# NoelShin/PixelPick

Measured on AMD Instinct MI355X. Metric: train_step_throughput, higher is better.
Workload: dtype f32; 1 GPU; BASELINE configs[1]: Cityscapes 256x512, C=19, DeepLabv3+-MobileNetV2; train step per-GPU batch 4 with 20 labelled px/img + Adam; acquisition entropy top-k=20, B=256 images/launch/GPU, NCHW fp32 logits; global_batch=4

## Files before the change

include/pixelpick_hip_knobs.h:

```cpp
#ifndef PIXELPICK_HIP_KNOBS_H
#define PIXELPICK_HIP_KNOBS_H

void pp_debug_set_reduce_mode(int mode);
void pp_debug_set_exact_formula(int on);
void pp_debug_set_acq_tuning(int occ, int ppt);
void pp_debug_set_dw_variant(int v);
void pp_debug_set_splitk(int v);
void pp_debug_set_wgrad_target(int blocks);
void pp_debug_set_bn_target(int blocks);
void pp_debug_set_bn_bytes_per_block(int bytes);
void pp_debug_set_bn_probe(void* device_buffer);
void pp_debug_set_conv_thresholds(int v);
void pp_debug_conv_plan(int64_t M, int Cn, int Ck, int ntaps, int* out4);
void pp_debug_set_conv_rows(int bits);
void pp_debug_set_conv_bn_fuse(int bits);
void pp_debug_set_x3_variant(int v);
void pp_debug_set_gemm_pw(int v);
void pp_debug_set_x3f(int v);
void pp_debug_set_x3(int on);
void pp_debug_set_conv_variant(int v);
int pp_debug_launch_log(char* buf, int n);


int pp_debug_occupy_cus(int blocks, const int* stop, uint64_t max_ticks, uint64_t* started, pp_stream_t stream);


#endif
```

pixelpick_amd/_lib.py:

```python
import ctypes
import os
import struct

import torch

_HERE = os.path.dirname(os.path.abspath(__file__))
LIB_PATH = os.path.join(_HERE, "libpixelpick_hip.so")
KNOBS_LIB_PATH = os.path.join(_HERE, "libpixelpick_hip_knobs.so")
_use_knobs = [os.environ.get("PIXELPICK_KNOBS_BUILD", "0") not in ("", "0")]


def use_knobs_build(on: bool = True):
    if _lib is not None and _use_knobs[0] != bool(on):
        raise PixelPickHipError("use_knobs_build() after the library was loaded")
    _use_knobs[0] = bool(on)


def knobs_build() -> bool:
    return _use_knobs[0]

_i64, _p, _int, _sz, _f = ctypes.c_int64, ctypes.c_void_p, ctypes.c_int, ctypes.c_size_t, ctypes.c_float
_u64 = ctypes.c_uint64

SIGNATURES = {
# ... 83 lines not shown
    "pp_bilinear_bwd": (_int, [_p, _i64, _int, _int, _int, _int, _p, _i64, _int, _int, _int, _f, _f, _int, _p, _sz, _p]),
    "pp_image_colsum": (_int, [_p, _i64, _int, _i64, _int, _f, _p, _i64, _p]),
    "pp_image_broadcast": (_int, [_p, _i64, _int, _i64, _int, _f, _p, _i64, _p]),
    "pp_dropout": (_int, [_p, _i64, _p, _i64, _i64, _int, _f, ctypes.c_uint64, _p, _p]),
    "pp_dropout2d": (_int, [_p, _i64, _p, _i64, _int, _i64, _int, _f, ctypes.c_uint64, _p, _p]),
    "pp_aug_resample_h": (_int, [_p, _int, _int, _p, _p, _int, _int, _p, _p]),
    "pp_aug_vcrop": (_int, [_p, _p, _p] + [_int] * 11 + [_p, _p]),
    "pp_aug_labels": (_int, [_p, _p, _int, _p, _p, _p, _p] + [_int] * 8 + [_p, _p, _p]),
    "pp_aug_jitter": (_int, [_p, _i64, _int, _f, _p, _p]),
    "pp_aug_blur": (_int, [_p, _int, _int, _p, _int, _p, _p]),
    "pp_aug_blur_q8": (_int, [_p, _int, _int, _p, _int, _p, _p]),
    "pp_aug_to_tensor": (_int, [_p, _i64, ctypes.POINTER(_f), ctypes.POINTER(_f), _p, _p]),
    "pp_sparse_ce_workspace_bytes": (_sz, []),
    "pp_sparse_ce_fwd_bwd": (_int, [_p, _int, _int, _i64, _i64, _i64, _p, _int, _p, _p, _p, _p, _p, _sz, _p]),
    "pp_sparse_ce_lowres_workspace_bytes": (_sz, []),
    "pp_sparse_ce_lowres_fwd_bwd": (_int, [_p, _i64] + [_int] * 7 + [_p, _int, _p, _p, _p, _p, _i64, _p, _sz, _p]),
    "pp_confusion_matrix_update": (_int, [_p, _int, _int, _i64, _i64, _i64, _p, _p, _p]),
    "pp_adam_step_flat": (_int, [_p, _p, _p, _p, _i64, _i64, _f, _f, _f, _f, _f, _f, _i64, _f, _p, _p]),
    "pp_sgd_step_flat": (_int, [_p, _p, _p, _i64, _i64, _f, _f, _f, _f, _i64, _f, _p, _p]),
    "pp_add2d": (_int, [_p, _i64, _p, _i64, _p, _i64, _i64, _int, _p]),
    "pp_nhwc_to_nchw": (_int, [_p, _i64, _int, _int, _i64, _p, _p]),
    "pp_nchw_to_nhwc": (_int, [_p, _int, _int, _i64, _p, _i64, _p]),
    "pp_bn_fused_capacity": (_int, []),
    "pp_yardstick_stream_read": (_int, [_p, _sz, _int, _p, _p]),
    "pp_yardstick_mfma_stream": (_int, [_int, _int, _p, _p]),
    "pp_set_kernel_events": (None, [_p, _p, _int]),
    "pp_set_comm_cu_reserve": (None, [_int]),
    "pp_get_comm_cu_reserve": (_int, []),
    "pp_plan_create": (_p, []),
    "pp_plan_destroy": (None, [_p]),
    "pp_plan_size": (_i64, [_p]),
    "pp_plan_entry_args": (_int, [_p]),
    "pp_plan_add_call": (_int, [_p, _p, _p, _int]),
    "pp_plan_add_event_record": (_int, [_p, _p, _p]),
    "pp_plan_add_stream_wait": (_int, [_p, _p, _p]),
    "pp_plan_add_join": (_int, [_p, _p, _p]),
    "pp_plan_add_host_break": (_int, [_p]),
    "pp_plan_replay": (_int, [_p, _i64, ctypes.POINTER(_i64)]),
}

KNOB_SIGNATURES = {
    "pp_debug_set_reduce_mode": (None, [_int]),
    "pp_debug_set_exact_formula": (None, [_int]),
    "pp_debug_set_acq_tuning": (None, [_int, _int]),
    "pp_debug_set_dw_variant": (None, [_int]),
    "pp_debug_set_splitk": (None, [_int]),
    "pp_debug_set_wgrad_target": (None, [_int]),
    "pp_debug_set_bn_target": (None, [_int]),
    "pp_debug_set_bn_bytes_per_block": (None, [_int]),
    "pp_debug_set_bn_probe": (None, [_p]),
    "pp_debug_set_conv_thresholds": (None, [_int]),
    "pp_debug_conv_plan": (None, [_i64, _int, _int, _int, _p]),
    "pp_debug_set_conv_variant": (None, [_int]),
    "pp_debug_set_conv_rows": (None, [_int]),
    "pp_debug_set_conv_bn_fuse": (None, [_int]),
    "pp_debug_set_x3": (None, [_int]),
    "pp_debug_set_x3f": (None, [_int]),
    "pp_debug_set_gemm_pw": (None, [_int]),
    "pp_debug_set_x3_variant": (None, [_int]),
    "pp_debug_occupy_cus": (_int, [_int, _p, _u64, _p, _p]),
    "pp_debug_launch_log": (_int, [ctypes.c_char_p, _int]),
}

_lib = None
knob_epoch = [0]


def _knob_setter(fn):
    def setter(*args):
        knob_epoch[0] += 1
        return fn(*args)
    setter.__name__ = getattr(fn, "__name__", "pp_debug_set")
    setter.__wrapped__ = fn
    return setter


class PixelPickHipError(RuntimeError):
    pass


def _preload_torch_hip():
    tl = os.path.join(os.path.dirname(torch.__file__), "lib", "libamdhip64.so")
    if os.path.exists(tl):
        ctypes.CDLL(tl, mode=ctypes.RTLD_GLOBAL)


def lib():
    global _lib
    if _lib is None:
        path = KNOBS_LIB_PATH if _use_knobs[0] else LIB_PATH
        if not os.path.exists(path):
            raise PixelPickHipError(
                f"{path} not found: build the HIP extension first "
                f"(python -m pixelpick_amd.build, or __graft_entry__.build()). No fallback path exists.")
        _preload_torch_hip()
        L = ctypes.CDLL(path)
        sigs = dict(SIGNATURES)
        if _use_knobs[0]:
            sigs.update(KNOB_SIGNATURES)
        for name, (res, args) in sigs.items():
            fn = getattr(L, name)
            fn.restype = res
            fn.argtypes = args
            if name.startswith(("pp_debug_set_", "pp_set_comm")):
                setattr(L, name, _knob_setter(fn))
        _lib = L
# ... 256 lines not shown
```

pixelpick_amd/csrc/conv_igemm.hip:

```cpp
#include <atomic>
#include <type_traits>

#include "pp_common.h"
#include "bn_xchg.h"
#include "conv_types.h"

namespace pp {


static int g_conv_xcd_remap = 1;
static int g_conv_novec = 0;
static int g_conv_lds_pad = 0;
static int g_conv_variant = 0;

typedef float f32x16s __attribute__((ext_vector_type(16)));
constexpr int BK = 16;
struct __attribute__((packed, aligned(4))) StemF4 { float x, y, z, w; };
struct __attribute__((packed, aligned(4))) StemF3 { float x, y, z; };
struct __attribute__((packed, aligned(4))) StemF2 { float x, y; };


template <int TM, int TN, bool A_MK, bool B_NK, int PITCH_A, int PITCH_B, int BKT = BK>
__device__ __forceinline__ void mma_step(const float* As, const float* Bs, int a_row0, int b_col0, f32x16 (&acc)[TM][TN])
{
    const int lane = threadIdx.x & 63;
    const int l31 = lane & 31, h = lane >> 5;
    constexpr int NQ = BKT / 8;
    float a[NQ][TM][4], b[NQ][TN][4];
#pragma unroll
    for (int q = 0; q < NQ; ++q) {
        const int k0 = 8 * q + 4 * h;
#pragma unroll
        for (int tm = 0; tm < TM; ++tm) {
            const int r = a_row0 + tm * 32 + l31;
            if constexpr (A_MK) {
                const float4 v = *reinterpret_cast<const float4*>(As + r * PITCH_A + k0);
                a[q][tm][0] = v.x; a[q][tm][1] = v.y; a[q][tm][2] = v.z; a[q][tm][3] = v.w;
            } else {
#pragma unroll
                for (int j = 0; j < 4; ++j) a[q][tm][j] = As[(k0 + j) * PITCH_A + r];
            }
        }
#pragma unroll
        for (int tn = 0; tn < TN; ++tn) {
            const int c = b_col0 + tn * 32 + l31;
            if constexpr (B_NK) {
                const float4 v = *reinterpret_cast<const float4*>(Bs + c * PITCH_B + k0);
                b[q][tn][0] = v.x; b[q][tn][1] = v.y; b[q][tn][2] = v.z; b[q][tn][3] = v.w;
            } else {
#pragma unroll
                for (int j = 0; j < 4; ++j) b[q][tn][j] = Bs[(k0 + j) * PITCH_B + c];
            }
// ... 555 lines not shown
        }
    }
    const int64_t m0 = (int64_t)mt * BM;
    const int n0 = nt * BN;
    unsigned tag0 = 0;
    if constexpr (BNF) tag0 = tag_issue(p.bn.sync);
    const float* zero = g_zero16;
    asm volatile("" : "+v"(zero));
    const uint32_t lds0 = __builtin_amdgcn_readfirstlane((uint32_t)(uintptr_t)smem);

    int a_e0[PA], a_c[PA];
    unsigned a_vm[PA];
#pragma unroll
    for (int i = 0; i < PA; ++i) {
        const int row = (wave * PA + i) * 16 + (lane >> 2);
        a_c[i] = ((lane & 3) ^ ((row >> 2) & 3)) * 4;
        const int64_t m = m0 + row;
        a_e0[i] = 0;
        a_vm[i] = 0u;
        if (m < p.M) {
            const unsigned mu = (unsigned)m;
            const unsigned t = mu / (unsigned)p.Wo;
            const int ow = (int)(mu - t * (unsigned)p.Wo);
            const unsigned bb = t / (unsigned)p.Ho;
            const int oh = (int)(t - bb * (unsigned)p.Ho);
            const int ih0 = oh * p.stride, iw0 = ow * p.stride;
            a_e0[i] = (((int)bb * p.H + ih0) * p.W + iw0) * (int)p.ldx + a_c[i];
            for (int t2 = 0; t2 < p.taps.n; ++t2) {
                const int ih = ih0 + p.taps.dh[t2], iw = iw0 + p.taps.dw[t2];
                a_vm[i] |= ((unsigned)ih < (unsigned)p.H && (unsigned)iw < (unsigned)p.W) ? (1u << t2) : 0u;
            }
        }
    }
    int b_e[PB], b_k[PB];
    bool b_ok[PB];
#pragma unroll
    for (int i = 0; i < PB; ++i) {
        const int P = (wave * PB + i) * 64 + lane;
        if constexpr (!BWD) {
            const int k = P / NQB, nq = ((P % NQB) - 8 * ((k >> 2) & 1)) & (NQB - 1);
            b_k[i] = k;
            b_ok[i] = n0 + nq * 4 < p.Cout;
            b_e[i] = k * p.Cout + n0 + nq * 4;
        } else {
            const int row = P >> 2, kq = (P & 3) ^ ((row >> 2) & 3);
            b_k[i] = kq * 4;
            b_ok[i] = n0 + row < p.Cin;
            b_e[i] = (n0 + row) * p.Cout + kq * 4;
        }
    }

    const int nchunk = (p.Ck + BK - 1) / BK;
    const int nk = p.taps.n * nchunk;
    const int ks_beg = p.splits > 1 ? (int)blockIdx.y * p.ks_per_split : 0;
    const int ks_end = p.splits > 1 ? (ks_beg + p.ks_per_split < nk ? ks_beg + p.ks_per_split : nk) : nk;
    const int n = ks_end - ks_beg;

    __shared__ int s_tap[32][2];
    if (tid < p.taps.n) {
        s_tap[tid][0] = (p.taps.dh[tid] * p.W + p.taps.dw[tid]) * (int)p.ldx + (p.multi ? p.tap_coff[tid] : 0);
        s_tap[tid][1] = p.multi ? p.tap_woff[tid] : p.taps.widx[tid] * p.Cin * p.Cout;
    }
    __syncthreads();
    int is_ti, is_ch;
    if (p.tap_inner) { is_ch = ks_beg / p.taps.n; is_ti = ks_beg - is_ch * p.taps.n; }
    else             { is_ti = ks_beg / nchunk;   is_ch = ks_beg - is_ti * nchunk; }
    int te_a = s_tap[is_ti][0], te_b = s_tap[is_ti][1];

    int st_ti = 0, st_c0 = 0, st_aoff = 0, st_boff = 0;
    uint32_t st_la = 0;
    auto issue_begin = [&](int stage) {
        st_ti = is_ti;
        st_c0 = is_ch * BK;
        st_aoff = __builtin_amdgcn_readfirstlane(te_a) + st_c0;
        st_boff = __builtin_amdgcn_readfirstlane(te_b) + (BWD ? st_c0 : st_c0 * p.Cout);
        st_la = lds0 + (uint32_t)(stage * STAGE_FLOATS * 4);
    };
    auto issue_a = [&](int i) {
        const bool ok = ((a_vm[i] >> st_ti) & 1u) && (st_c0 + a_c[i] < p.Ck);
        const float* src = p.x + (size_t)(unsigned)(a_e0[i] + st_aoff);
        conv_glds16(ok ? src : zero, st_la + (uint32_t)((wave * PA + i) * 1024));
    };
    auto issue_b = [&](int i) {
        const bool ok = b_ok[i] && (st_c0 + b_k[i] < (BWD ? p.Cout : p.Cin));
        const float* src = p.w + (size_t)(unsigned)(b_e[i] + st_boff);
        conv_glds16(ok ? src : zero, st_la + (uint32_t)(BM * BK * 4 + (wave * PB + i) * 1024));
    };
    const bool tap_in = p.tap_inner != 0;
    const int inner_lim = tap_in ? p.taps.n : nchunk;
    auto a_src = [&](int i) -> const float* {
        const bool ok = ((a_vm[i] >> st_ti) & 1u) && (st_c0 + a_c[i] < p.Ck);
        return ok ? p.x + (size_t)(unsigned)(a_e0[i] + st_aoff) : zero;
    };
    auto b_src = [&](int i) -> const float* {
        const bool ok = b_ok[i] && (st_c0 + b_k[i] < (BWD ? p.Cout : p.Cin));
        return ok ? p.w + (size_t)(unsigned)(b_e[i] + st_boff) : zero;
    };
    auto issue_a_all = [&]() {
        if constexpr (PA == 2) conv_glds16x2(a_src(0), a_src(1), st_la + (uint32_t)(wave * PA * 1024));
        else issue_a(0);
    };
    auto issue_b_all = [&]() {
        if constexpr (PB == 2) conv_glds16x2(b_src(0), b_src(1), st_la + (uint32_t)(BM * BK * 4 + wave * PB * 1024));
        else issue_b(0);
    };
    auto issue_end = [&]() {
        int inner = (tap_in ? is_ti : is_ch) + 1, outer = tap_in ? is_ch : is_ti;
        const bool wrap = inner == inner_lim;
        inner = wrap ? 0 : inner;
        outer += wrap ? 1 : 0;
        is_ti = tap_in ? inner : outer;
        is_ch = tap_in ? outer : inner;
        const int tn = is_ti < p.taps.n ? is_ti : 0;
        te_a = s_tap[tn][0];
        te_b = s_tap[tn][1];
    };
    auto issue = [&](int stage) {
        issue_begin(stage);
#pragma unroll
        for (int i = 0; i < PA; ++i) issue_a(i);
#pragma unroll
        for (int i = 0; i < PB; ++i) issue_b(i);
        issue_end();
    };

    const int l31 = lane & 31, h = lane >> 5;
    const int swz = (l31 >> 2) & 3;
    auto read_a = [&](int stage, Frags& F, int q, int tm) {
        const float4* As4 = reinterpret_cast<const float4*>(smem + stage * STAGE_FLOATS);
        const int r = (wm * TM + tm) * 32 + l31;
        const float4 v = As4[r * 4 + ((2 * q + h) ^ swz)];
        F.a[q][tm][0] = v.x; F.a[q][tm][1] = v.y; F.a[q][tm][2] = v.z; F.a[q][tm][3] = v.w;
    };
    auto read_b = [&](int stage, Frags& F, int q, int tn) {
        const float* Bs = smem + stage * STAGE_FLOATS + BM * BK;
        const int c = (wn * TN + tn) * 32 + l31;
        if constexpr (BWD) {
            const float4 v = reinterpret_cast<const float4*>(Bs)[c * 4 + ((2 * q + h) ^ swz)];
            F.b[q][tn][0] = v.x; F.b[q][tn][1] = v.y; F.b[q][tn][2] = v.z; F.b[q][tn][3] = v.w;
        } else {
            const int cc = (c + 32 * h) & (BN - 1);
#pragma unroll
            for (int j = 0; j < 4; ++j) F.b[q][tn][j] = Bs[(8 * q + 4 * h + j) * BN + cc];
        }
    };
    auto read_frags = [&](int stage, Frags& F) {
#pragma unroll
        for (int q = 0; q < 2; ++q) {
#pragma unroll
            for (int t = 0; t < TM; ++t) read_a(stage, F, q, t);
#pragma unroll
            for (int t = 0; t < TN; ++t) read_b(stage, F, q, t);
        }
    };

    f32x16 acc[TM][TN];
#pragma unroll
    for (int i = 0; i < TM; ++i)
#pragma unroll
        for (int j = 0; j < TN; ++j)
#pragma unroll
            for (int r = 0; r < 16; ++r) acc[i][j][r] = 0.0f;

    auto mma4 = [&](const Frags& F, int q, int j) {
#pragma unroll
        for (int tm = 0; tm < TM; ++tm)
// ... 2312 lines not shown

static int g_conv_splitk = 1;
static int g_splitk_tiles = 192, g_splitk_target = 512, g_splitk_min_nk = 12, g_splitk_min_iters = 4;

static int g_conv_deepk = 1;
static int g_conv_ablate_reduce = 0;
static int g_conv_dma = 1;
static int g_conv_dma64 = 1;
static int g_conv_big_bk32 = 0;
static int g_conv_n64 = 1;
static int g_conv_tap_inner = 1;
static int g_conv_bwd_rows = 1;
static int64_t g_rows_fwd_min = 16384;
static int g_direct_rows_max = 4096;
static int g_conv_ksplit = 1, g_ksplit_k_min = 256;
static int g_bwd_phases = 1;
static int g_shortk64 = 1;
static int g_big_tile_min = 384, g_wgrad_rows_min = 128;

static ConvPlan plan_conv(int64_t M, int Cn, int Ck, int ntaps, bool vec = true)
{
    ConvPlan pl{};
    const int64_t mt128 = cdiv(M, 128), mt64 = cdiv(M, 64);
    if (Cn <= 32) {
        pl.cfg = 0; pl.n_tiles = 1; pl.tiles = mt128;
    } else if (Cn > 64 && mt128 * cdiv(Cn, 128) >= g_big_tile_min && !(g_shortk64 && ntaps == 1 && Ck <= 256)) {
        pl.cfg = 1;
        const int rem = Cn % 128;
        pl.bn64 = g_conv_variant == 2 || (g_conv_n64 && rem != 0 && rem <= 64 && (cdiv(Cn, 128) * 128 - Cn) * 100 > 15 * Cn);
        pl.n_tiles = (int)cdiv(Cn, pl.bn64 ? 64 : 128);
        pl.tiles = mt128 * pl.n_tiles;
        if (g_conv_big_bk32 && !pl.bn64 && vec && Ck >= 64) pl.cfg = 4;
    } else {
        pl.cfg = 2; pl.n_tiles = (int)cdiv(Cn, 64); pl.tiles = mt64 * pl.n_tiles;
        if (g_conv_deepk && !g_conv_dma64 && vec && Ck >= 256 && M >= 4096) pl.cfg = 3;
    }
    const int bk = pl.cfg == 3 ? 64 : (pl.cfg == 4 ? 32 : BK);
    const int nk = ntaps * (int)cdiv(Ck, bk);
    pl.splits = 1;
    pl.ks_per_split = nk;
    if (g_conv_splitk && pl.tiles < g_splitk_tiles && nk >= (pl.cfg == 3 ? 4 : g_splitk_min_nk)) {
        int64_t s = cdiv(g_splitk_target, pl.tiles);
        const int min_iters = pl.cfg == 3 ? 2 : g_splitk_min_iters;
        if (s > nk / min_iters) s = nk / min_iters;
        if (s > 32) s = 32;
        if (s > 1) {
            pl.ks_per_split = (int)cdiv(nk, s);
            pl.splits = (int)cdiv(nk, pl.ks_per_split);
        }
    }
    return pl;
}

static bool ksplit_shape_ok(int64_t M, int Cn, int Ck, int ntaps, int stride)
{
    return g_conv_ksplit && ntaps == 1 && stride == 1 && M <= g_direct_rows_max && Ck >= g_ksplit_k_min && Cn >= 32 && Cn <= 512 &&
           Ck % 4 == 0 && Cn % 4 == 0;
}

static int64_t splitk_stats_rows_per_block(int64_t M) { return M >= 8192 ? 64 : 16; }

static int64_t conv_stats_rows(const ConvPlan& pl, int64_t M, int Cn)
{
    if (pl.splits > 1) {
        if (Cn % 4 != 0 || Cn / 4 > 256) return 0;
        return cdiv(M, splitk_stats_rows_per_block(M));
    }
    if (pl.cfg == 0) return cdiv(M, 128) * 4;
    if (pl.cfg == 1 || pl.cfg == 4) return cdiv(M, 128) * 2;
    return cdiv(M, 64) * 2;
}

static int g_conv_x3 = 1;
static int g_x3_var = 0;
struct X3Plan { bool ok, classic, f32; int Kp; int64_t rows_a, a_plane, b_rows, b_plane; size_t bytes, b_off; };
static int g_conv_x3_mid = 1;
static double g_x3_mid_flop = 16e9, g_x3w_flop = 8e9;
static int g_x3_mid_tiles = 256;
static int g_x3f = 0;
static double g_x3f_flop = 1e9;
static int g_x3f_tiles = 128, g_x3f_k = 256;
static X3Plan x3_plan(const ConvPlan& pl, int64_t M, int64_t rows_a, int Ck, int n_rows, int ntaps_w, int ntaps_live, bool vec)
{
    X3Plan x{};
    const int64_t t128 = cdiv(M, 128) * cdiv(n_rows, 128);
    const double flop = 2.0 * (double)M * n_rows * ntaps_live * Ck;
    const bool mid = g_conv_x3_mid && pl.cfg == 2 && t128 >= g_x3_mid_tiles && flop >= g_x3_mid_flop;
    if (!g_conv_x3 || !vec || ntaps_live > 32) return x;
    x.classic = (pl.cfg == 1 || mid) && pl.splits <= 1 && (int64_t)ntaps_live * Ck >= 512;
    const int64_t t64 = n_rows % 64 == 0 ? cdiv(M, 128) * (n_rows / 64) : 0;
    x.f32 = g_x3f && n_rows >= 64 && (x.classic || (flop >= g_x3f_flop && (int64_t)ntaps_live * Ck >= g_x3f_k &&
                                                    std::max(t128, t64) >= g_x3f_tiles && (pl.cfg == 1 || pl.cfg == 2 || pl.cfg == 3 || pl.cfg == 4)));
    if (!x.classic && !x.f32) return x;
    x.Kp = (int)cdiv(Ck, 16) * 16;
    x.rows_a = rows_a;
    x.a_plane = (rows_a + 1) * x.Kp;
    x.b_rows = (int64_t)ntaps_w * n_rows;
    x.b_plane = (x.b_rows + 1) * x.Kp;
    if (x.b_plane * 2 >= (1ll << 32) - 4096) { x.classic = x.f32 = false; return x; }
    if (x.a_plane * 2 >= (1ll << 32) - 4096) x.classic = false;
    if (!x.classic && !x.f32) return x;
    x.b_off = x.classic ? align_up((size_t)3 * x.a_plane * 2, 256) : 0;
    x.bytes = x.b_off + align_up((size_t)3 * x.b_plane * 2, 256);
    x.ok = true;
    return x;
}
// ... 327 lines not shown
#define PP_KSPLIT_AFF(TM_, TN_, NST_) hipLaunchKernelGGL((conv1x1_ksplit_dma_kernel<TM_, TN_, NST_, false, true>), grid, dim3(kThreads), 0, st, p)
        if (!BWD && p.in_scale) {
            if (kc.tm == 1 && kc.tn == 1) PP_KSPLIT_AFF(1, 1, 4);
            else if (kc.tm == 2)          PP_KSPLIT_AFF(2, 1, 3);
            else                          PP_KSPLIT_AFF(1, 2, 3);
        } else
        if (kc.tm == 1 && kc.tn == 1) PP_KSPLIT(1, 1, 5);
        else if (kc.tm == 2)          PP_KSPLIT(2, 1, 3);
        else                          PP_KSPLIT(1, 2, 3);
#undef PP_KSPLIT_AFF
#undef PP_KSPLIT
        return check_launch("conv1x1_ksplit_dma_kernel");
    }
    p.tap_inner = g_conv_tap_inner;
    p.n_tiles = pl.n_tiles;
    p.splits = pl.splits;
    p.ks_per_split = pl.ks_per_split;
    p.part = reinterpret_cast<float*>(workspace);
    dim3 grid((unsigned)pl.tiles, (unsigned)pl.splits);
    const char* kname = "conv_igemm_kernel<128x32>";
    if (pl.cfg == 0) {
        if (vec) hipLaunchKernelGGL((conv_igemm_kernel<128, 32, 4, 1, BWD, true>), grid, dim3(kThreads), 0, st, p);
        else     hipLaunchKernelGGL((conv_igemm_kernel<128, 32, 4, 1, BWD, false>), grid, dim3(kThreads), 0, st, p);
    } else if (pl.cfg == 1) {
        if (pl.bn64) {
            const bool dma_ok64 = vec && g_conv_dma && (!BWD || g_conv_dma == 1 || g_conv_dma == 3) && p.taps.n <= 32 && (!BWD || p.bwd_stride <= 1) &&
                                  (int64_t)p.B * p.H * p.W * p.ldx < (1ll << 31) - (1ll << 24) &&
                                  (int64_t)kMaxTaps * p.Cin * p.Cout < (1ll << 31);
            kname = dma_ok64 ? "conv_igemm_dma_kernel<128x64>" : "conv_igemm_kernel<128x64>";
            if (dma_ok64) hipLaunchKernelGGL((conv_igemm_dma_kernel<128, 64, BWD>), grid, dim3(kThreads), 0, st, p);
            else
            if (vec) hipLaunchKernelGGL((conv_igemm_kernel<128, 64, 2, 2, BWD, true>), grid, dim3(kThreads), 0, st, p);
            else     hipLaunchKernelGGL((conv_igemm_kernel<128, 64, 2, 2, BWD, false>), grid, dim3(kThreads), 0, st, p);
        } else {
            const bool dma_ok = vec && g_conv_dma && (!BWD || g_conv_dma == 1) && p.taps.n <= 32 && (!BWD || p.bwd_stride <= 1) &&
                                (int64_t)p.B * p.H * p.W * p.ldx < (1ll << 31) - (1ll << 24) &&
                                (int64_t)kMaxTaps * p.Cin * p.Cout < (1ll << 31);
            kname = dma_ok ? "conv_igemm_dma_kernel<128x128>" : "conv_igemm_kernel<128x128>";
            if (dma_ok) hipLaunchKernelGGL((conv_igemm_dma_kernel<128, 128, BWD>), grid, dim3(kThreads), 0, st, p);
            else if (vec) hipLaunchKernelGGL((conv_igemm_kernel<128, 128, 2, 2, BWD, true>), grid, dim3(kThreads), g_conv_lds_pad, st, p);
            else     hipLaunchKernelGGL((conv_igemm_kernel<128, 128, 2, 2, BWD, false>), grid, dim3(kThreads), g_conv_lds_pad, st, p);
        }
    } else if (pl.cfg == 4) {
        kname = "conv_igemm_kernel<128x128 bk32>";
        hipLaunchKernelGGL((conv_igemm_kernel<128, 128, 2, 2, BWD, true, 32>), grid, dim3(kThreads), 0, st, p);
    } else if (pl.cfg == 3) {
        kname = "conv_igemm_kernel<64x64 bk64>";
        hipLaunchKernelGGL((conv_igemm_kernel<64, 64, 2, 2, BWD, true, 64>), grid, dim3(kThreads), 0, st, p);
    } else {
        const bool dma_ok = vec && g_conv_dma64 && (!BWD || g_conv_dma64 == 1) && p.taps.n <= 32 && (!BWD || p.bwd_stride <= 1) &&
                            (int64_t)p.B * p.H * p.W * p.ldx < (1ll << 31) - (1ll << 24) &&
                            (int64_t)kMaxTaps * p.Cin * p.Cout < (1ll << 31);
        kname = dma_ok ? "conv_igemm_dma_kernel<64x64>" : "conv_igemm_kernel<64x64>";
        if (dma_ok)   hipLaunchKernelGGL((conv_igemm_dma_kernel<64, 64, BWD>), grid, dim3(kThreads), 0, st, p);
        else if (vec) hipLaunchKernelGGL((conv_igemm_kernel<64, 64, 2, 2, BWD, true>), grid, dim3(kThreads), 0, st, p);
        else          hipLaunchKernelGGL((conv_igemm_kernel<64, 64, 2, 2, BWD, false>), grid, dim3(kThreads), 0, st, p);
    }
    if (int rc = check_launch(kname)) return rc;
    if (pl.splits > 1 && p.stats) {
        const int64_t rpb = splitk_stats_rows_per_block(p.M);
        hipLaunchKernelGGL(splitk_reduce_stats_kernel, dim3((unsigned)cdiv(p.M, rpb)), dim3(256), 0, st, p.part, pl.splits, p.M, p.Cn,
                           p.bias, p.y, p.ldy, p.accumulate, p.stats, rpb);
        return check_launch("splitk_reduce_stats_kernel");
    }
    if (pl.splits > 1 && !(g_conv_ablate_reduce & (BWD ? 2 : 1))) {
        const bool plain = p.epi.gamma == nullptr && p.epi.res == nullptr && p.epi.act == 0 && p.Cn % 4 == 0 && p.ldy % 4 == 0;
        int64_t nb = cdiv(plain ? p.M * (p.Cn / 4) : p.M * p.Cn, 256);
        if (nb > 8192) nb = 8192;
        hipLaunchKernelGGL(splitk_reduce_kernel, dim3((unsigned)nb), dim3(256), 0, st, p.part, pl.splits, p.M, p.Cn, p.bias,
                           p.y, p.ldy, p.epi, p.accumulate);
        return check_launch("splitk_reduce_kernel");
    }
    return PP_OK;
}

static int g_narrow_rows_min = 16, g_narrow_splits_max = 4096;
static int64_t narrow_splits_max(int64_t floats_per_split)
{
    int64_t s = (16ll << 20) / (floats_per_split * 4);
    if (s > g_narrow_splits_max) s = g_narrow_splits_max;
    if (s < 1024) s = 1024;
    return s;
}
static int g_wgrad_narrow = 1;
static int g_wgrad_stem = 1;
static int g_wgrad_m64 = 1;
static int g_wgrad_xcd = 1;
static int g_wgrad_dma = 1;
static const int g_wgrad_lds_pad_default = 0;
static int g_wgrad_lds_pad = 0;
static int g_wgrad_target = 1024;
static int g_wgrad_balance = 1;
static int g_wgrad_fold = 0;
static int* wgrad_counters_take(int n)
{
    static std::atomic<uint32_t> next{0};
    static int* base = nullptr;
    if (!base) {
        void* q = nullptr;
        if (hipGetSymbolAddress(&q, HIP_SYMBOL(g_wgrad_counters)) != hipSuccess) { (void)hipGetLastError(); return nullptr; }
        base = reinterpret_cast<int*>(q);
    }
    uint32_t at;
    for (;;) {
        uint32_t cur = next.load(std::memory_order_relaxed);
        at = (cur + (uint32_t)n > (uint32_t)kWgradCounters) ? 0u : cur;
// ... 106 lines not shown
        else if (p.Cout == 24)  hipLaunchKernelGGL((wgrad_narrow_out_kernel<24, 4>), grid, blk, 0, st, p, NL, RL, rows_per_split);
        else                    hipLaunchKernelGGL((wgrad_narrow_out_kernel<32, 4>), grid, blk, 0, st, p, NL, RL, rows_per_split);
    }
    if (int rc = check_launch(kname)) return rc;
    if (reduce_deferrable(job, p.taps, cn, splits, dbias)) {
        fill_reduce_job(job, 2, p.part, dw, cn, splits, p.taps);
        *bias_done = true;
        return PP_OK;
    }
    hipLaunchKernelGGL(wgrad_reduce_wide_kernel, dim3((unsigned)cdiv((int64_t)nt * cn, 8)), dim3(256), 0, st, p.part, (int)splits,
                       nt, cn, p.taps, dw);
    if (int rc = check_launch("wgrad_reduce_wide_kernel")) return rc;
    if (fuse_bias) {
        hipLaunchKernelGGL(bias_grad_final_kernel, dim3((unsigned)cdiv(p.Cout, 8)), dim3(256), 0, st, p.bias_part, (int)splits, p.Cout, dbias);
        if (int rc = check_launch("bias_grad_final_kernel")) return rc;
        *bias_done = true;
    }
    return 0;
}

static inline bool conv_geom_sane(int H, int W, int stride, int pad, int dil)
{
    return H <= (1 << 24) && W <= (1 << 24) && stride <= (1 << 16) && pad >= 0 && pad <= (1 << 20) && dil <= (1 << 16);
}

static int conv_common_check(const void* a, const void* b, const void* c, int B, int H, int W, int Cin, int Cout,
                             int kh, int kw, int stride, int pad, int dil)
{
    if (!a || !b || !c) return fail(PP_ERR_BAD_ARG, "conv: null pointer");
    if (B < 1 || H < 1 || W < 1 || Cin < 1 || Cout < 1) return fail(PP_ERR_BAD_ARG, "conv: bad shape");
    if (kh < 1 || kw < 1 || kh > kMaxTaps || kw > kMaxTaps || kh * kw > kMaxTaps) return fail(PP_ERR_UNSUPPORTED, "conv: kernel %dx%d unsupported", kh, kw);
    if (stride < 1 || dil < 1 || pad < 0 || !conv_geom_sane(H, W, stride, pad, dil)) return fail(PP_ERR_BAD_ARG, "conv: bad stride/dilation/padding");
    return PP_OK;
}

static inline int out_size(int in, int k, int stride, int pad, int dil) { return (in + 2 * pad - dil * (k - 1) - 1) / stride + 1; }

}

using namespace pp;

extern "C" {

#ifdef PP_DEBUG_KNOBS
void pp_debug_conv_plan(int64_t M, int Cn, int Ck, int ntaps, int* out)
{
    const ConvPlan pl = plan_conv(M, Cn, Ck, ntaps, Ck % 4 == 0 && Cn % 4 == 0);
    const int rows[5] = {128, 128, 64, 64, 128}, cols[5] = {32, pl.bn64 ? 64 : 128, 64, 64, 128};
    out[0] = rows[pl.cfg]; out[1] = cols[pl.cfg]; out[2] = (int)pl.tiles; out[3] = pl.splits;
}
#endif

#ifdef PP_DEBUG_KNOBS
void pp_debug_set_splitk(int v)
{
    g_splitk_tiles = (v & 1023) ? (v & 1023) : 192;
    g_splitk_target = ((v >> 10) & 1023) ? ((v >> 10) & 1023) : 512;
    g_splitk_min_nk = ((v >> 20) & 63) ? ((v >> 20) & 63) : 12;
    g_splitk_min_iters = ((v >> 26) & 15) ? ((v >> 26) & 15) : 4;
}
#endif

#ifdef PP_DEBUG_KNOBS
void pp_debug_set_conv_rows(int bits) { g_conv_bwd_rows = (bits & 1) ? 0 : 1; g_rows_fwd_min = (bits & 2) ? 65536 : 16384; }
#endif

#ifdef PP_DEBUG_KNOBS
void pp_debug_set_conv_bn_fuse(int bits) { g_conv_bn_fuse = bits & 15; }
#endif

int pp_yardstick_mfma_stream(int data_kind, int iters, float* sink, pp_stream_t stream)
{
    if (!sink || iters < 1 || data_kind < 0 || data_kind > 2) return fail(PP_ERR_BAD_ARG, "mfma_stream: bad argument");
    const dim3 grid((unsigned)device_cus()), block(512);
    hipStream_t st = as_stream(stream);
    EventScope ev(st);
    if (data_kind == 0) hipLaunchKernelGGL(mfma_stream_kernel<0>, grid, block, 0, st, sink, iters, 7u);
    else if (data_kind == 1) hipLaunchKernelGGL(mfma_stream_kernel<1>, grid, block, 0, st, sink, iters, 7u);
    else hipLaunchKernelGGL(mfma_stream_kernel<2>, grid, block, 0, st, sink, iters, 7u);
    return check_launch("mfma_stream_kernel");
}

#ifdef PP_DEBUG_KNOBS
void pp_debug_set_gemm_pw(int v)
{
    g_gemm_pw = (v & 15) <= 7 ? (v & 15) : 1;
    g_gemm_pw_rows_min = (v >> 4) > 0 ? (v >> 4) : 4096;
}
#endif
#ifdef PP_DEBUG_KNOBS
void pp_debug_set_x3f(int v)
{
    g_x3f = (v & 1) ? 1 : 0;
    static const double gf[8] = {1e9, 0.5e9, 2e9, 4e9, 8e9, 0.25e9, 0.0, 1e9};
    g_x3f_flop = gf[(v >> 1) & 7];
    static const int tl[4] = {128, 64, 192, 256};
    g_x3f_tiles = tl[(v >> 4) & 3];
    static const int kk[4] = {256, 128, 512, 16};
    g_x3f_k = kk[(v >> 6) & 3];
}
#endif
#ifdef PP_DEBUG_KNOBS
void pp_debug_set_x3_variant(int v) { g_x3_var = (v >= 0 && v <= 11) ? v : 0; }
#endif

#ifdef PP_DEBUG_KNOBS
// ... 454 lines not shown
            m.pl.ks_per_split = (int)cdiv(nk, sp);
            m.pl.splits = (int)cdiv(nk, m.pl.ks_per_split);
        }
    }
    m.ok = vec && m.pl.cfg == 2 && g_conv_dma64 == 1 && (int64_t)B * H * W * lddy < (1ll << 31) - (1ll << 24);
    return m;
}

size_t pp_conv2d_bwd_data_multi_workspace_bytes(int B, int H, int W, int Cin, int Cout, int nb, int k0, int d0, int k1, int d1, int k2, int d2,
                                                int k3, int d3)
{
    const int k[4] = {k0, k1, k2, k3}, d[4] = {d0, d1, d2, d3};
    const MultiBwd m = multi_bwd_setup(B, H, W, Cin, Cout, nb, k, d, (int64_t)nb * Cout);
    if (!m.ok) return 0;
    return align_up(m.pl.splits > 1 ? (size_t)m.pl.splits * m.p.M * Cin * 4 : 256, 256);
}

int pp_conv2d_bwd_data_multi(const float* dy, int64_t lddy, int B, int H, int W, int Cout, int nb, const float* w0, int k0, int d0,
                             const float* w1, int k1, int d1, const float* w2, int k2, int d2, const float* w3, int k3, int d3, float* dx,
                             int64_t lddx, int Cin, int accumulate, void* workspace, size_t ws_bytes, pp_stream_t stream)
{
    const int k[4] = {k0, k1, k2, k3}, d[4] = {d0, d1, d2, d3};
    const float* w[4] = {w0, w1, w2, w3};
    if (!dy || !dx || lddy < (int64_t)nb * Cout || lddx < Cin) return fail(PP_ERR_BAD_ARG, "conv bwd_data multi: null / leading dimension");
    MultiBwd m = multi_bwd_setup(B, H, W, Cin, Cout, nb, k, d, lddy);
    if (!m.ok) return fail(PP_ERR_UNSUPPORTED, "conv bwd_data multi: not offered for this shape (ask the workspace query first)");
    const float* base = nullptr;
    for (int b = 0; b < nb; ++b) {
        if (!w[b]) return fail(PP_ERR_BAD_ARG, "conv bwd_data multi: null weight");
        if (!base || w[b] < base) base = w[b];
    }
    if ((reinterpret_cast<uintptr_t>(dy) & 15) || (reinterpret_cast<uintptr_t>(dx) & 15) || lddx % 4 != 0)
        return fail(PP_ERR_BAD_ARG, "conv bwd_data multi: dy / dx must be 16-byte aligned");
    ConvParams& p = m.p;
    for (int t = 0; t < p.taps.n; ++t) {
        const int b = p.taps.widx[t] >> 8, lt = p.taps.widx[t] & 255;
        const int64_t off = (w[b] - base) + (int64_t)lt * Cin * Cout;
        if ((reinterpret_cast<uintptr_t>(w[b]) & 15) || off + (int64_t)Cin * Cout >= (1ll << 31))
            return fail(PP_ERR_UNSUPPORTED, "conv bwd_data multi: the branch weights must be 16-byte aligned and within 8 GiB of each other");
        p.tap_woff[t] = (int)off;
        p.taps.widx[t] = 0;
    }
    const size_t need = m.pl.splits > 1 ? (size_t)m.pl.splits * p.M * Cin * 4 : 0;
    if (need && (!workspace || ws_bytes < need)) return fail(PP_ERR_WORKSPACE, "conv bwd_data multi: workspace %zu < %zu", ws_bytes, need);
    hipStream_t st = as_stream(stream);
    EventScope ev(st);
    p.x = dy; p.w = base; p.bias = nullptr; p.y = dx; p.ldy = lddx; p.accumulate = accumulate ? 1 : 0;
    p.xcd_remap = g_conv_xcd_remap;
    p.tap_inner = g_conv_tap_inner;
    p.n_tiles = m.pl.n_tiles;
    p.splits = m.pl.splits;
    p.ks_per_split = m.pl.ks_per_split;
    p.part = reinterpret_cast<float*>(workspace);
    hipLaunchKernelGGL((conv_igemm_dma_kernel<64, 64, true>), dim3((unsigned)m.pl.tiles, (unsigned)m.pl.splits), dim3(kThreads), 0, st, p);
    if (int rc = check_launch("conv_igemm_dma_kernel<multi>")) return rc;
    if (m.pl.splits > 1) {
        int64_t nblk = cdiv(p.M * (p.Cn / 4), 256);
        if (nblk > 8192) nblk = 8192;
        hipLaunchKernelGGL(splitk_reduce_kernel, dim3((unsigned)nblk), dim3(256), 0, st, p.part, m.pl.splits, p.M, p.Cn, p.bias, p.y, p.ldy, p.epi,
                           p.accumulate);
        return check_launch("splitk_reduce_kernel");
    }
    return PP_OK;
}

size_t pp_x3_planes_bytes(int64_t rows, int C)
{
    if (rows < 1 || C < 1) return 0;
    return align_up((size_t)3 * (size_t)(rows + 1) * (size_t)(cdiv(C, 16) * 16) * 2, 256);
}

int pp_x3_split(const float* x, int64_t ldx, int64_t rows, int C, void* planes, size_t planes_bytes, pp_stream_t stream)
{
    if (!x || !planes || rows < 1 || C < 1) return fail(PP_ERR_BAD_ARG, "x3_split: null / empty");
    if (C % 4 != 0 || ldx % 4 != 0 || (reinterpret_cast<uintptr_t>(x) & 15) || (reinterpret_cast<uintptr_t>(planes) & 255))
        return fail(PP_ERR_BAD_ARG, "x3_split: C and ld must be multiples of 4, x 16-byte and planes 256-byte aligned");
    const int Kp = (int)cdiv(C, 16) * 16;
    const int64_t plane = (rows + 1) * Kp;
    if (plane * 2 >= (1ll << 32) - 4096) return fail(PP_ERR_UNSUPPORTED, "x3_split: plane of %lld bytes", (long long)(plane * 2));
    if (planes_bytes < pp_x3_planes_bytes(rows, C)) return fail(PP_ERR_WORKSPACE, "x3_split: planes buffer");
    const int64_t ta = (rows + 1) * (Kp / 8);
    hipLaunchKernelGGL(x3_split_kernel, dim3((unsigned)std::min<int64_t>(cdiv(ta, 256), 4096)), dim3(256), 0, as_stream(stream), x, ldx, rows, C,
                       reinterpret_cast<uint16_t*>(planes), Kp, plane);
    return check_launch("x3_split_kernel");
}

static bool conv_bn_bwd_shape(ConvParams& p, ConvPlan& pl, int B, int H, int W, int Cin, int Cout, int kh, int kw, int stride, int pad, int dil,
                              int64_t lddy, int* R_out)
{
    if (B < 1 || H < 1 || W < 1 || Cin < 1 || Cout < 1 || kh < 1 || kw < 1 || kh > kMaxTaps || kw > kMaxTaps || kh * kw > kMaxTaps || !conv_geom_sane(H, W, stride, pad, dil) || stride != 1 || dil < 1) return false;
    const int Ho = out_size(H, kh, stride, pad, dil), Wo = out_size(W, kw, stride, pad, dil);
    if (Ho < 1 || Wo < 1) return false;
    p = ConvParams{};
    p.ldx = lddy; p.B = B; p.H = Ho; p.W = Wo; p.Ho = H; p.Wo = W; p.Ck = Cout; p.Cn = Cin; p.Cin = Cin; p.Cout = Cout;
    p.stride = 1; p.M = (int64_t)B * H * W; p.bwd_stride = 1;
    build_taps(p.taps, kh, kw, 1, pad, dil, Ho, Wo, H, W, true, 1);
    if (p.M > 0x7FFFFFFFll || p.taps.n == 0) return false;
    const bool vec = Cin % 4 == 0 && Cout % 4 == 0 && lddy % 4 == 0;
    pl = plan_conv(p.M, Cin, Cout, p.taps.n, vec);
    const BnFusePlan f = bn_fuse_plan_bwd(p, pl, vec);
    if (R_out) *R_out = f.R;
    return f.kind != 0;
}

int pp_conv2d_bwd_data_bn_bwd_ok(int B, int H, int W, int Cin, int Cout, int kh, int kw, int stride, int pad, int dil)
{
// ... 345 lines not shown
```

pixelpick_amd/csrc/conv_types.h:

```cpp
#pragma once
#include "pp_common.h"
#include "bn_xchg.h"

namespace pp {

typedef float f32x16 __attribute__((ext_vector_type(16)));
constexpr int kThreads = 256;
constexpr int kMaxTaps = 49;

struct ConvTaps {
    int n;
    int dh[kMaxTaps];
    int dw[kMaxTaps];
    int widx[kMaxTaps];
};

struct BnTrain {
    const float* gamma; const float* beta; float eps, momentum;
    float* running_mean; float* running_var; float* mean; float* invstd;
    const float* res; int64_t ldr; int act;
    float* y; int64_t ldy;
    xword* part; int* sync; int R;
    const float* bx; int64_t ldbx; float* dgamma; float* dbeta;
    const float* gin; int64_t ldgin; float* dres; int64_t lddr;
};

struct ConvParams {
    const uint16_t* a_pre;
    const uint16_t* b_pre;
    const float* x;
    const float* w;
    const float* bias;
    float* y;
    int64_t ldx, ldy;
    int B, H, W;
    int Ho, Wo;
    int Ck;
    int Cn;
    int Cin, Cout;
    int stride;
    int64_t M;
    int bwd_stride;
    int n_tiles;
    int xcd_remap;
    int splits;
    int ks_per_split;
    float* part;
    Epilogue epi;
    int accumulate;
    int tap_inner;
    const float* in_scale;
    const float* in_shift;
    int in_act;
    int multi;
    int tap_coff[32], tap_woff[32];
    BnTrain bn;
    float* stats;
    ConvTaps taps;
};

template <int TM, int TN>
__device__ __forceinline__ void conv_epilogue(const ConvParams& p, f32x16 (&acc)[TM][TN], int64_t m0, int n0, int wm, int wn)
{
    const int tid = threadIdx.x;
    const int lane = tid & 63, l31 = lane & 31, hh = lane >> 5;
#pragma unroll
    for (int tn = 0; tn < TN; ++tn) {
        const int n = n0 + (wn * TN + tn) * 32 + l31;
        if (n >= p.Cn) continue;
        const bool final_pass = p.splits <= 1;
        const float bv = (p.bias && final_pass) ? p.bias[n] : 0.0f;
        const bool affine = final_pass && p.epi.gamma != nullptr;
        float sc = 1.0f, sf = 0.0f;
        if (affine) {
            const float is = 1.0f / sqrtf(p.epi.var[n] + p.epi.eps);
            sc = p.epi.gamma[n] * is;
            sf = p.epi.beta[n] - p.epi.mean[n] * sc;
        }
        const float* res = final_pass ? p.epi.res : nullptr;
        const int act = final_pass ? p.epi.act : 0;
        float* out = p.splits > 1 ? p.part + (int64_t)blockIdx.y * p.M * p.Cn : p.y;
        const int64_t ldo = p.splits > 1 ? (int64_t)p.Cn : p.ldy;
        float s1 = 0.0f, s2 = 0.0f;
#pragma unroll
        for (int tm = 0; tm < TM; ++tm) {
#pragma unroll
            for (int r = 0; r < 16; ++r) {
                const int64_t m = m0 + (wm * TM + tm) * 32 + (r & 3) + 8 * (r >> 2) + 4 * hh;
                if (m < p.M) {
                    float o = acc[tm][tn][r] + bv;
                    if (affine) o = fmaf(o, sc, sf);
                    if (res) o += res[m * p.epi.ldr + n];
                    if (final_pass && p.accumulate) o += out[m * ldo + n];
                    o = epi_act(o, act);
                    out[m * ldo + n] = o;
                    s1 += o;
                    s2 = fmaf(o, o, s2);
                }
            }
        }
        if (p.stats && final_pass) {
            s1 += __shfl_xor(s1, 32, 64);
            s2 += __shfl_xor(s2, 32, 64);
            if (hh == 0) {
                const int64_t pr = m0 / (TM * 32) + wm;
                p.stats[(pr * 2 + 0) * p.Cn + n] = s1;
                p.stats[(pr * 2 + 1) * p.Cn + n] = s2;
            }
        }
// ... 28 lines not shown
```

Baseline: 755.2 images/s.

## Skip dead convolution taps per tile in DMA implicit-GEMM kernel

Adds per-tile tap pruning to the DMA implicit-GEMM conv kernel. Each block ORs the per-row tap-validity masks to find which taps touch any in-bounds input, compacts the tap table to only those taps, and remaps the K-loop and split-K ranges onto the compacted index space. A host-side scan over the M tiles turns pruning on only when the busiest tile uses at most 90% of the taps, which in practice means large-dilation convs like ASPP on small feature maps. The goal is to stop issuing zero-filled loads and MFMA steps for taps that fall entirely in padding, at the cost of extra syncs, an atomic, a host-side per-launch scan, and more complex index arithmetic.

```diff
diff --git a/include/pixelpick_hip_knobs.h b/include/pixelpick_hip_knobs.h
--- a/include/pixelpick_hip_knobs.h
+++ b/include/pixelpick_hip_knobs.h
@@ -19,6 +19,7 @@
 void pp_debug_set_x3f(int v);
 void pp_debug_set_x3(int on);
 void pp_debug_set_conv_variant(int v);
+void pp_debug_set_conv_prune(int v);
 int pp_debug_launch_log(char* buf, int n);
 
 
diff --git a/pixelpick_amd/_lib.py b/pixelpick_amd/_lib.py
--- a/pixelpick_amd/_lib.py
+++ b/pixelpick_amd/_lib.py
@@ -159,6 +159,7 @@
     "pp_debug_set_conv_thresholds": (None, [_int]),
     "pp_debug_conv_plan": (None, [_i64, _int, _int, _int, _p]),
     "pp_debug_set_conv_variant": (None, [_int]),
+    "pp_debug_set_conv_prune": (None, [_int]),
     "pp_debug_set_conv_rows": (None, [_int]),
     "pp_debug_set_conv_bn_fuse": (None, [_int]),
     "pp_debug_set_x3": (None, [_int]),
diff --git a/pixelpick_amd/csrc/conv_igemm.hip b/pixelpick_amd/csrc/conv_igemm.hip
--- a/pixelpick_amd/csrc/conv_igemm.hip
+++ b/pixelpick_amd/csrc/conv_igemm.hip
@@ -1,3 +1,4 @@
+#include <algorithm>
 #include <atomic>
 #include <type_traits>
 
@@ -659,18 +660,51 @@
 
     const int nchunk = (p.Ck + BK - 1) / BK;
     const int nk = p.taps.n * nchunk;
-    const int ks_beg = p.splits > 1 ? (int)blockIdx.y * p.ks_per_split : 0;
-    const int ks_end = p.splits > 1 ? (ks_beg + p.ks_per_split < nk ? ks_beg + p.ks_per_split : nk) : nk;
-    const int n = ks_end - ks_beg;
+    int ks_beg = p.splits > 1 ? (int)blockIdx.y * p.ks_per_split : 0;
+    int ks_end = p.splits > 1 ? (ks_beg + p.ks_per_split < nk ? ks_beg + p.ks_per_split : nk) : nk;
 
     __shared__ int s_tap[32][2];
-    if (tid < p.taps.n) {
-        s_tap[tid][0] = (p.taps.dh[tid] * p.W + p.taps.dw[tid]) * (int)p.ldx + (p.multi ? p.tap_coff[tid] : 0);
-        s_tap[tid][1] = p.multi ? p.tap_woff[tid] : p.taps.widx[tid] * p.Cin * p.Cout;
-    }
+    __shared__ unsigned s_live;
+    int ntl = p.taps.n;
+    if (p.prune) {
+        if (tid == 0) s_live = 0u;
+        __syncthreads();
+        unsigned any = 0u;
+#pragma unroll
+        for (int i = 0; i < PA; ++i) any |= a_vm[i];
+        if (any) atomicOr(&s_live, any);
+        __syncthreads();
+        const unsigned live = __builtin_amdgcn_readfirstlane(s_live);
+        ntl = __popc(live);
+        if (tid < p.taps.n && ((live >> tid) & 1u)) {
+            const int j = __popc(live & ((1u << tid) - 1u));
+            s_tap[j][0] = (p.taps.dh[tid] * p.W + p.taps.dw[tid]) * (int)p.ldx + (p.multi ? p.tap_coff[tid] : 0);
+            s_tap[j][1] = p.multi ? p.tap_woff[tid] : p.taps.widx[tid] * p.Cin * p.Cout;
+        }
+#pragma unroll
+        for (int i = 0; i < PA; ++i) {
+            unsigned c = 0u;
+            int j = 0;
+            for (int t = 0; t < p.taps.n; ++t)
+                if ((live >> t) & 1u) { c |= ((a_vm[i] >> t) & 1u) << j; ++j; }
+            a_vm[i] = c;
+        }
+        auto live_before = [&](int k) { return (k / p.taps.n) * ntl + __popc(live & ((1u << (k % p.taps.n)) - 1u)); };
+        ks_beg = live_before(ks_beg);
+        ks_end = live_before(ks_end);
+    } else {
+        if (tid < p.taps.n) {
+            s_tap[tid][0] = (p.taps.dh[tid] * p.W + p.taps.dw[tid]) * (int)p.ldx + (p.multi ? p.tap_coff[tid] : 0);
+            s_tap[tid][1] = p.multi ? p.tap_woff[tid] : p.taps.widx[tid] * p.Cin * p.Cout;
+        }
+    }
+    ntl = __builtin_amdgcn_readfirstlane(ntl);
+    ks_beg = __builtin_amdgcn_readfirstlane(ks_beg);
+    ks_end = __builtin_amdgcn_readfirstlane(ks_end);
+    const int n = ks_end > ks_beg ? ks_end - ks_beg : 0;
     __syncthreads();
     int is_ti, is_ch;
-    if (p.tap_inner) { is_ch = ks_beg / p.taps.n; is_ti = ks_beg - is_ch * p.taps.n; }
+    if (p.tap_inner) { is_ch = ntl > 0 ? ks_beg / ntl : 0; is_ti = ks_beg - is_ch * ntl; }
     else             { is_ti = ks_beg / nchunk;   is_ch = ks_beg - is_ti * nchunk; }
     int te_a = s_tap[is_ti][0], te_b = s_tap[is_ti][1];
 
@@ -694,7 +728,7 @@
         conv_glds16(ok ? src : zero, st_la + (uint32_t)(BM * BK * 4 + (wave * PB + i) * 1024));
     };
     const bool tap_in = p.tap_inner != 0;
-    const int inner_lim = tap_in ? p.taps.n : nchunk;
+    const int inner_lim = tap_in ? ntl : nchunk;
     auto a_src = [&](int i) -> const float* {
         const bool ok = ((a_vm[i] >> st_ti) & 1u) && (st_c0 + a_c[i] < p.Ck);
         return ok ? p.x + (size_t)(unsigned)(a_e0[i] + st_aoff) : zero;
@@ -718,7 +752,7 @@
         outer += wrap ? 1 : 0;
         is_ti = tap_in ? inner : outer;
         is_ch = tap_in ? outer : inner;
-        const int tn = is_ti < p.taps.n ? is_ti : 0;
+        const int tn = is_ti < ntl ? is_ti : 0;
         te_a = s_tap[tn][0];
         te_b = s_tap[tn][1];
     };
@@ -3137,6 +3171,39 @@
     return pl;
 }
 
+static int g_conv_prune = 1;
+
+static unsigned rows_live_mask(const ConvParams& p, int64_t m0, int64_t m1)
+{
+    const unsigned all = p.taps.n >= 32 ? 0xffffffffu : ((1u << p.taps.n) - 1u);
+    unsigned live = 0u;
+    for (int64_t m = m0; m < m1 && live != all;) {
+        const int64_t img_row = m / p.Wo;
+        const int ow0 = (int)(m - img_row * p.Wo);
+        const int oh = (int)(img_row % p.Ho);
+        const int64_t e = std::min<int64_t>(m1, m + (p.Wo - ow0));
+        const int ow1 = ow0 + (int)(e - m) - 1;
+        for (int t = 0; t < p.taps.n; ++t) {
+            const int ih = oh + p.taps.dh[t];
+            if (ih >= 0 && ih < p.H && std::max(ow0 + p.taps.dw[t], 0) <= std::min(ow1 + p.taps.dw[t], p.W - 1)) live |= 1u << t;
+        }
+        m = e;
+    }
+    return live;
+}
+
+static void prune_setup(ConvParams& p)
+{
+    p.prune = 0;
+    const int64_t tiles_m = cdiv(p.M, 64);
+    if (!g_conv_prune || p.stride != 1 || p.bwd_stride > 1 || !p.tap_inner || p.taps.n < 2 || p.taps.n > 32 || tiles_m > 8192 || p.bn.part)
+        return;
+    int busiest = 0;
+    for (int64_t t = 0; t < tiles_m && busiest * 10 <= p.taps.n * 9; ++t)
+        busiest = std::max(busiest, __builtin_popcount(rows_live_mask(p, t * 64, std::min<int64_t>(p.M, t * 64 + 64))));
+    p.prune = busiest * 10 <= p.taps.n * 9 ? 1 : 0;
+}
+
 static bool ksplit_shape_ok(int64_t M, int Cn, int Ck, int ntaps, int stride)
 {
     return g_conv_ksplit && ntaps == 1 && stride == 1 && M <= g_direct_rows_max && Ck >= g_ksplit_k_min && Cn >= 32 && Cn <= 512 &&
@@ -3570,6 +3637,7 @@
                             (int64_t)p.B * p.H * p.W * p.ldx < (1ll << 31) - (1ll << 24) &&
                             (int64_t)kMaxTaps * p.Cin * p.Cout < (1ll << 31);
         kname = dma_ok ? "conv_igemm_dma_kernel<64x64>" : "conv_igemm_kernel<64x64>";
+        if (dma_ok) prune_setup(p);
         if (dma_ok)   hipLaunchKernelGGL((conv_igemm_dma_kernel<64, 64, BWD>), grid, dim3(kThreads), 0, st, p);
         else if (vec) hipLaunchKernelGGL((conv_igemm_kernel<64, 64, 2, 2, BWD, true>), grid, dim3(kThreads), 0, st, p);
         else          hipLaunchKernelGGL((conv_igemm_kernel<64, 64, 2, 2, BWD, false>), grid, dim3(kThreads), 0, st, p);
@@ -3782,6 +3850,13 @@
 #endif
 
 #ifdef PP_DEBUG_KNOBS
+void pp_debug_set_conv_prune(int v)
+{
+    g_conv_prune = v ? 1 : 0;
+}
+#endif
+
+#ifdef PP_DEBUG_KNOBS
 void pp_debug_set_splitk(int v)
 {
     g_splitk_tiles = (v & 1023) ? (v & 1023) : 192;
@@ -4342,6 +4417,7 @@
     p.splits = m.pl.splits;
     p.ks_per_split = m.pl.ks_per_split;
     p.part = reinterpret_cast<float*>(workspace);
+    prune_setup(p);
     hipLaunchKernelGGL((conv_igemm_dma_kernel<64, 64, true>), dim3((unsigned)m.pl.tiles, (unsigned)m.pl.splits), dim3(kThreads), 0, st, p);
     if (int rc = check_launch("conv_igemm_dma_kernel<multi>")) return rc;
     if (m.pl.splits > 1) {
diff --git a/pixelpick_amd/csrc/conv_types.h b/pixelpick_amd/csrc/conv_types.h
--- a/pixelpick_amd/csrc/conv_types.h
+++ b/pixelpick_amd/csrc/conv_types.h
@@ -55,6 +55,7 @@
     int multi;
     int tap_coff[32], tap_woff[32];
     BnTrain bn;
+    int prune;
     float* stats;
     ConvTaps taps;
 };
```

After: 756.5 images/s (median of 6 runs). No clear change (+0.2%).
